# marthinwurer/gcmiipy

Measured on AMD Instinct MI355X. Metric: cell-updates/s (C-grid Matsuno step), higher is better.
Workload: dtype f64; 1 GPU; 2-D shallow water + theta + viscosity + van-Leer tracer, 4096x2048 fp64 (BASELINE configs[2]); variant=fused, decomposition=1 latitude band(s)

## Files before the change

### gcmiipy_amd/_lib.py

```python
import ctypes as C
import os

_HERE = os.path.dirname(os.path.abspath(__file__))
LIB_PATH = os.environ.get("GCMCORE_LIB", os.path.join(_HERE, "lib", "libgcmcore.so"))

ABI_VERSION = 1

SW2D, SW2D_TEMP, PE2D, PE25D = 1, 2, 3, 4
P, U, V, T, Q = 0, 1, 2, 3, 4
TRACER_NONE, TRACER_UPWIND, TRACER_VANLEER = 0, 1, 2
VARIANT_AUTO, VARIANT_STAGED, VARIANT_FUSED = 0, 1, 2
F64, F32 = 0, 1
MAX_TRACERS = 16
TRACER_STATS_WORDS = 6
CLIM_WORDS3, CLIM_WORDS2 = 10, 2
SW2D_PLAN_WORDS = 9
PHASE_HELD_SUAREZ, PHASE_MOIST, PHASE_CLIMATE, PHASE_TRACER_FORCING = range(4)
PHASE_PLAN_WORDS = 5
ADV_UPWIND, ADV_FV_UPWIND, ADV_FV_PLAIN, ADV_VANLEER, ADV_MOMENTUM = range(5)
DIAG_ANY_NAN, DIAG_MAX_U, DIAG_MEAN_P, DIAG_SUM_P, DIAG_MIN_U, DIAG_MAX_V, DIAG_MIN_V = range(7)
DIAG_TV_P, DIAG_TV_U, DIAG_TV_V, DIAG_TV_T, DIAG_TV_Q = range(7, 12)
INT_SPU, INT_PIT, INT_PN, INT_PHI, INT_PGFU = range(5)
FL_VAN_LEER, FL_CALC_R, FL_DONOR_FLUX, FL_DONOR_ADVECTION = range(4)
OP1D_ADVEC_Q, OP1D_CALC_PU, OP1D_UN_PU, OP1D_ADVEC_P, OP1D_ADVEC_PU, OP1D_ADVEC_T, OP1D_PGF = range(7)
# ... 63 lines not shown
class TracerForcing(C.Structure):
    _fields_ = [("source", C.c_double), ("decay", C.c_double), ("pin_value", C.c_double),
                ("emission", _dp), ("pin_mask", C.POINTER(C.c_ubyte))]


_H = C.c_void_p
SYMBOLS = {
    "gcm_abi_version": (C.c_int, []),
    "gcm_device_count": (C.c_int, []),
    "gcm_build_info": (C.c_char_p, []),
    "gcm_exner_table": (C.c_int, [_dp]),
    "gcm_filter_plan": (C.c_int, [C.c_int, C.POINTER(C.c_uint), C.c_int]),
    "gcm_create": (C.c_int, [C.POINTER(Config), C.POINTER(_H)]),
    "gcm_destroy": (C.c_int, [_H]),
    "gcm_last_error": (C.c_char_p, [_H]),
    "gcm_set_state": (C.c_int, [_H] + [C.c_void_p] * 5),
    "gcm_get_state": (C.c_int, [_H] + [C.c_void_p] * 5),
    "gcm_members": (C.c_int, [_H]),
    "gcm_set_member": (C.c_int, [_H, C.c_int] + [C.c_void_p] * 5),
    "gcm_get_member": (C.c_int, [_H, C.c_int] + [C.c_void_p] * 5),
    "gcm_diag_members": (C.c_int, [_H, C.c_int, _dp, C.c_int]),
    "gcm_step": (C.c_int, [_H, C.c_int, C.c_double]),
    "gcm_sw2d_plan": (C.c_int, [_H, C.c_int, C.POINTER(C.c_int), C.c_int]),
    "gcm_pe25d_phase_geometry": (C.c_int, [C.c_int] * 7 + [C.POINTER(C.c_int), C.c_int]),
    "gcm_pe25d_phase_plan": (C.c_int, [_H, C.c_int, C.c_int, C.c_int, C.POINTER(C.c_int), C.c_int]),
    "gcm_half_step": (C.c_int, [_H, C.c_int, C.c_double]),
    "gcm_end_step": (C.c_int, [_H, C.c_double]),
    "gcm_end_step_begin": (C.c_int, [_H, C.c_double]),
    "gcm_end_step_finish": (C.c_int, [_H, C.c_double]),
    "gcm_get_star": (C.c_int, [_H] + [C.c_void_p] * 5),
    "gcm_set_star": (C.c_int, [_H] + [C.c_void_p] * 5),
    "gcm_diag": (C.c_int, [_H, C.c_int, _dp]),
    "gcm_energy": (C.c_int, [_H, _dp, C.c_int, _dp]),
    "gcm_stats": (C.c_int, [_H, _dp, C.c_int, _dp]),
    "gcm_flux_limiter": (C.c_int, [C.c_int, C.c_int, C.c_void_p, C.c_void_p, C.c_double, C.c_double, C.c_void_p]),
    "gcm_polar_filter": (C.c_int, [_H, C.c_int, C.c_void_p, C.c_void_p]),
    "gcm_get_intermediate": (C.c_int, [_H, C.c_int, C.c_void_p]),
    "gcm_set_ground": (C.c_int, [_H, C.c_void_p]),
    "gcm_get_ground": (C.c_int, [_H, C.c_void_p]),
    "gcm_grey_radiation": (C.c_int, [_H] + [C.c_double] * 4 + [_dp, _dp, C.c_void_p, C.c_void_p]),
    "gcm_solar_step": (C.c_int, [_H] + [C.c_double] * 5 + [_dp, _dp]),
    "gcm_set_physics": (C.c_int, [_H, C.c_void_p]),
    "gcm_get_utc": (C.c_int, [_H, _dp]),
    "gcm_set_held_suarez": (C.c_int, [_H, C.POINTER(HeldSuarez)]),
    "gcm_held_suarez_on": (C.c_int, [_H]),
    "gcm_held_suarez_step": (C.c_int, [_H, C.c_double, C.POINTER(HeldSuarez)]),
# ... 117 lines not shown
```

### gcmiipy_amd/core.py

```python
import collections
import ctypes as C

import numpy as np

from . import _lib
from ._lib import lib


class GcmError(RuntimeError):
    pass


def _check(rc, h=None):
    if rc == _lib.OK:
        return
    msg = lib.gcm_last_error(h).decode() if (h or rc) else ""
    if rc == _lib.ERR_ARG:
        raise ValueError(msg or "gcmcore: bad argument")
    raise GcmError("gcmcore error %d: %s" % (rc, msg))


def _count(n, h):
    if n < 0:
        _check(n, h)
# ... 539 lines not shown
                out[i] = k
        return out

    def set_tracer_scheme(self, scheme):
        scheme = tracer_scheme_id(scheme)
        _check(lib.gcm_set_tracer_scheme(self._h, scheme), self._h)
        self.options["tracer_scheme"] = scheme

    @property
    def tracer_scheme(self):
        return _count(lib.gcm_tracer_scheme(self._h), self._h)

    @property
    def band_tracer_rows(self):
        return _count(lib.gcm_band_tracer_rows(self._h), self._h)

    @property
    def tracer_count(self):
        return _count(lib.gcm_tracer_count(self._h), self._h)

    def step(self, nsteps, dt):
        _check(lib.gcm_step(self._h, int(nsteps), float(dt)), self._h)

    def sw2d_plan(self, nsteps):
        out = (C.c_int * _lib.SW2D_PLAN_WORDS)()
        _check(lib.gcm_sw2d_plan(self._h, int(nsteps), out, _lib.SW2D_PLAN_WORDS), self._h)
        return dict(variant={_lib.VARIANT_FUSED: "fused", _lib.VARIANT_STAGED: "staged"}[out[0]],
                    rows_per_band=out[1], cols=out[2], strip=out[3], strip2=out[4], two_step_launches=out[5],
                    single_step_launches=out[6], preload=bool(out[7]), stream=bool(out[8]))

    def phase_plan(self, phase, rows=None, accumulate=True):
        out = (C.c_int * _lib.PHASE_PLAN_WORDS)()
        _check(lib.gcm_pe25d_phase_plan(self._h, phase_id(phase), -1 if rows is None else int(rows), int(bool(accumulate)),
                                        out, _lib.PHASE_PLAN_WORDS), self._h)
        return _phase_dict(phase_id(phase), out)

    def half_step(self, stage, dt):
        _check(lib.gcm_half_step(self._h, int(stage), float(dt)), self._h)

    def end_step(self, dt):
        _check(lib.gcm_end_step(self._h, float(dt)), self._h)

    def end_step_begin(self, dt):
        _check(lib.gcm_end_step_begin(self._h, float(dt)), self._h)

    def end_step_finish(self, dt):
# ... 323 lines not shown
```

### gcmiipy_amd/csrc/gcm_handle.h

```cpp
#pragma once
#include "../../include/gcmcore.h"

#include <hip/hip_runtime.h>

#include <algorithm>
#include <cstdio>
#include <string>
#include <vector>

#include "pe25d_kernels.h"
#include "sw2d_kernels.h"

struct GcmBandExchange {
    gcm_exchange xch{};
    bool set = false, primed = false;
    bool inflight = false;
    bool overlap = false;
    hipEvent_t ev_pack = nullptr, ev_comm = nullptr;
    bool join_pending = false;
    bool on_comm = false;
};

struct GcmTiming {
    bool on = false;
// ... 19 lines not shown
    hipStream_t stream = nullptr;
    std::string err;
    std::vector<void *> allocs;

    double *cur[GCM_NFIELDS] = {}, *nxt[GCM_NFIELDS] = {}, *star[GCM_NFIELDS] = {};
    double *geo = nullptr, *irho = nullptr, *sst = nullptr, *qtmp = nullptr;
    bool has[GCM_NFIELDS] = {};
    double *exner_tab = nullptr;
    int G = gcm::kGhost;
    int since_exchange = 0;
    bool ghosts_current = false;
    bool star_valid = false;
    bool launch_refused = false;
    hipStream_t comm = nullptr;
    double *snap[GCM_NFIELDS] = {};
    int snap_since_exchange = 0;
    int variant = GCM_VARIANT_FUSED;
    int rows_per_band = 32;
    int M = 1;
    long mstride = 0;
    bool f32 = false;
    int esz = 8;
    int cols = 1;
    double *staging = nullptr;
    int staging_members = 0;

    double *diag_dev = nullptr;
    static constexpr int kDiagBlocks = 512;

    GcmTiming time;
    gcm::Pe25d *pe = nullptr;
    GcmBandExchange band;
    GcmPhases phases;
};

#define HIPCHK(h, call)                                                                    \
    do {                                                                                   \
        hipError_t e_ = (call);                                                            \
        if (e_ != hipSuccess) {                                                            \
            char b_[512];                                                                  \
            snprintf(b_, sizeof b_, "%s failed: %s (%s:%d)", #call, hipGetErrorString(e_), \
                     __FILE__, __LINE__);                                                  \
            (h)->err = b_;                                                                 \
            return GCM_ERR_HIP;                                                            \
        }                                                                                  \
    } while (0)
// ... 53 lines not shown
```

### gcmiipy_amd/csrc/gcmcore.hip

```cpp
#include <cmath>
#include <cstdlib>
#include <cstring>

#include "gcm_handle.h"

using namespace gcm;

std::string &gcm_create_error() {
    thread_local std::string e;
    return e;
}

static int alloc_field(gcm_handle *h, double **p) {
    static const long skew_unit = getenv("GCM_ALLOC_SKEW") ? atol(getenv("GCM_ALLOC_SKEW")) : 256;
    const size_t n = all_members_elems(h);
    const size_t skew = (size_t)(skew_unit > 0 ? skew_unit : 0) * (h->allocs.size() % 16) / h->esz;
    void *d = nullptr;
    HIPCHK(h, hipMalloc(&d, (n + skew) * h->esz));
    HIPCHK(h, hipMemsetAsync(d, 0, (n + skew) * h->esz, h->stream));
    h->allocs.push_back(d);
    *p = at(h, (double *)d, (long)(skew + (size_t)h->G * h->W));
    return GCM_OK;
}

// ... 109 lines not shown
            if (cfg->tracer < 0 || cfg->tracer > GCM_TRACER_VANLEER)
                return bail(GCM_ERR_ARG, "gcm_create: bad tracer");
            h->has[GCM_U] = h->has[GCM_V] = h->has[GCM_P] = true;
            h->has[GCM_T] = temp;
            h->has[GCM_Q] = temp && cfg->tracer != GCM_TRACER_NONE;
            h->variant = cfg->variant == GCM_VARIANT_AUTO ? GCM_VARIANT_FUSED : cfg->variant;
            if (h->variant != GCM_VARIANT_FUSED && h->variant != GCM_VARIANT_STAGED)
                return bail(GCM_ERR_ARG, "gcm_create: bad variant");
            for (int f = 0; f < GCM_NFIELDS; ++f) {
                if (!h->has[f]) continue;
                if ((rc = alloc_field(h, &h->cur[f]))) return bail(rc, "");
                if ((rc = alloc_field(h, &h->nxt[f]))) return bail(rc, "");
                if (f != GCM_Q && (rc = alloc_field(h, &h->star[f]))) return bail(rc, "");
            }
            if (temp) {
                if ((rc = alloc_field(h, &h->geo))) return bail(rc, "");
                if ((rc = alloc_field(h, &h->irho))) return bail(rc, "");
                if ((rc = alloc_field(h, &h->sst))) return bail(rc, "");
            }
            if (h->has[GCM_Q] && (rc = alloc_field(h, &h->qtmp))) return bail(rc, "");
            if (temp && !upload_exner_table(h)) return bail(GCM_ERR_HIP, "gcm_create: exner table upload failed");
            const int tr = h->has[GCM_Q] ? cfg->tracer : 0;
            if (h->f32) h->cols = sw2d_fused_cols<float>(h->W, h->H, temp, tr, h->wrap, h->M);
            h->rows_per_band = h->f32 ? sw2d_fused_rows_per_band<float>(h->W, h->H, temp, tr, h->wrap, h->M, h->cols)
                                      : sw2d_fused_rows_per_band<double>(h->W, h->H, temp, tr, h->wrap, h->M);
            break;
        }
        case GCM_PE2D: {
            if (!(cfg->dx > 0)) return bail(GCM_ERR_ARG, "gcm_create: dx must be > 0");
            if (cfg->nranks != 1)
                return bail(GCM_ERR_UNSUPPORTED, "gcm_create: GCM_PE2D has no latitude-band mode");
            h->variant = GCM_VARIANT_STAGED;
            for (int f = 0; f < GCM_NFIELDS; ++f) {
                h->has[f] = true;
                if ((rc = alloc_field(h, &h->cur[f]))) return bail(rc, "");
                if ((rc = alloc_field(h, &h->nxt[f]))) return bail(rc, "");
                if ((rc = alloc_field(h, &h->star[f]))) return bail(rc, "");
            }
            if (!upload_exner_table(h)) return bail(GCM_ERR_HIP, "gcm_create: exner table upload failed");
            break;
        }
        case GCM_PE25D: {
            std::string msg;
            h->pe = pe25d_create(*cfg, h->stream, &msg);
            if (!h->pe) return bail(msg.find("hip") == 0 ? GCM_ERR_HIP : GCM_ERR_ARG, msg);
            h->has[GCM_P] = h->has[GCM_U] = h->has[GCM_V] = h->has[GCM_T] = h->has[GCM_Q] = true;
            break;
        }
// ... 123 lines not shown
    a.inv_dx2 = 1.0 / (h->cfg.dx * h->cfg.dx);
    a.h_dx = 0.5 / h->cfg.dx;
    a.dtdx = dt / h->cfg.dx;
    a.g_dx = 9.8 / h->cfg.dx;
    a.mu_dx2 = (18.5 * 1e-6) * 287.0 / (h->cfg.dx * h->cfg.dx);
    a.inv_dx2_ = a.inv_dx2;
    return a;
}

static void run_derive(const gcm_handle *h, const Sw2dArgs &a, hipStream_t s) {
    if (h->f32) launch_sw2d_derive(narrow_args(a), s);
    else launch_sw2d_derive(a, s);
}
static void run_stage(const gcm_handle *h, const Sw2dArgs &a, bool temp, hipStream_t s) {
    if (h->f32) launch_sw2d_stage(narrow_args(a), temp, s);
    else launch_sw2d_stage(a, temp, s);
}
static void run_tracer_axis(const gcm_handle *h, const Sw2dArgs &a, int axis, bool limit, const double *q_in,
                            double *q_out, hipStream_t s) {
    if (h->f32) launch_tracer_axis(narrow_args(a), axis, limit, (const float *)q_in, (float *)q_out, s);
    else launch_tracer_axis(a, axis, limit, q_in, q_out, s);
}
static bool run_fused(const gcm_handle *h, const Sw2dArgs &a, bool temp, int tracer, hipStream_t s) {
    return h->f32 ? launch_sw2d_fused(narrow_args(a), temp, tracer, s, h->cols) : launch_sw2d_fused(a, temp, tracer, s);
}
static bool run_fused2(const gcm_handle *h, const Sw2dArgs &a, hipStream_t s) {
    return h->f32 ? launch_sw2d_fused2(narrow_args(a), s) : launch_sw2d_fused2(a, s);
}

int launch_status(gcm_handle *h) {
    const hipError_t e = hipGetLastError();
    if (h->launch_refused) {
        h->launch_refused = false;
        return fail(h, GCM_ERR_HIP, std::string("sw2d fused kernel: launch refused") +
                                        (e != hipSuccess ? std::string(": ") + hipGetErrorString(e) : std::string()));
    }
    HIPCHK(h, e);
    return GCM_OK;
}

void swap_state(gcm_handle *h) {
    for (int f = 0; f < GCM_NFIELDS; ++f) std::swap(h->cur[f], h->nxt[f]);
    h->ghosts_current = false;
}

static void tick(gcm_handle *h, hipStream_t s) {
    if (h->time.on && h->time.used < h->time.ev.size()) (void)hipEventRecord(h->time.ev[h->time.used++], s);
// ... 104 lines not shown
                h->launch_refused = true;
                return launch_status(h);
            }
            swap_state(h);
            n0 += 2;
        }
    }
    for (int n = n0; n < nsteps; ++n) {
        const int e = step_extra_rows(h);
        step_rows(h, dt, -e, h->H + e, h->stream);
        swap_state(h);
        if (!h->wrap) ++h->since_exchange;
    }
    h->star_valid = false;
    return launch_status(h);
}

int gcm_sw2d_plan(gcm_handle *h, int nsteps, int *out, int nout) {
    if (!h || h->pe || nsteps < 0 || !out || nout < GCM_SW2D_PLAN_WORDS) return GCM_ERR_ARG;
    const bool fused = h->variant == GCM_VARIANT_FUSED;
    const bool temp = h->cfg.model == GCM_SW2D_TEMP;
    const int pairs = steps_in_pairs(h) ? nsteps / 2 : 0;
    const int e = step_extra_rows(h);
    Sw2dFusedForm f{false, false};
    if (fused)
        f = sw2d_fused_form(temp, h->has[GCM_Q] ? h->cfg.tracer : 0, h->rows_per_band, h->W, h->H + 2 * e, h->M, h->esz);
    out[0] = h->variant;
    out[1] = fused ? h->rows_per_band : 0;
    out[2] = fused ? h->cols : 0;
    out[3] = fused ? sw2d_fused_strip_cols(h->cols) : 0;
    out[4] = fused ? kStrip2Cols : 0;
    out[5] = pairs;
    out[6] = nsteps - 2 * pairs;
    out[7] = f.preload;
    out[8] = f.stream;
    return GCM_OK;
}

int gcm_step_interior(gcm_handle *h, double dt, void *stream) {
    if (!h) return GCM_ERR_ARG;
    if (h->pe) return pe25d_step_part(h->pe, 0, dt, (hipStream_t)stream, &h->err);
    if (h->wrap) return fail(h, GCM_ERR_STATE, "step_interior: handle is not a latitude band");
    if (h->G != kGhost) return fail(h, GCM_ERR_STATE, "step_interior: halo_steps > 1 steps through gcm_step");
    step_rows(h, dt, kGhost, h->H - kGhost, (hipStream_t)stream);
    return launch_status(h);
}

int gcm_step_boundary(gcm_handle *h, double dt, void *stream) {
    if (!h) return GCM_ERR_ARG;
    if (h->pe) return pe25d_step_part(h->pe, 1, dt, (hipStream_t)stream, &h->err);
    if (h->wrap) return fail(h, GCM_ERR_STATE, "step_boundary: handle is not a latitude band");
    hipStream_t s = (hipStream_t)stream;
    if (h->H <= 2 * kGhost) {
        step_rows(h, dt, 0, h->H, s);
    } else {
        step_rows(h, dt, 0, kGhost, s);
        step_rows(h, dt, h->H - kGhost, h->H, s);
    }
    swap_state(h);
// ... 204 lines not shown
```

### gcmiipy_amd/csrc/sw2d_impl.h

```cpp
#pragma once
#include <hip/hip_runtime.h>

#include <cstdlib>
#include <type_traits>

#include "gcm_math.h"
#include "sw2d_kernels.h"

namespace gcm {

__device__ __forceinline__ long row_off(int j, int H, int W, bool wrap) {
    if (wrap) {
        j %= H;
        if (j < 0) j += H;
    }
    return (long)j * W;
}

template <typename T>
__device__ __forceinline__ Sw2dArgsT<T> member_args(const Sw2dArgsT<T> &a0, int m) {
    Sw2dArgsT<T> a = a0;
    const long o = (long)m * a0.mstride;
    auto mv = [o](auto *p) { return p ? p + o : p; };
    a.bu = mv(a.bu); a.bv = mv(a.bv); a.bp = mv(a.bp); a.bt = mv(a.bt); a.bq = mv(a.bq);
// ... 171 lines not shown
    t.du = adv_vel_u(R0.u, uw, ue, RM.u, RP.u, R0.v, vw, RP.v, vsw, h_dx) +
           geo_grad(ge, R0.g, g_dx);
    t.dv = adv_vel_v(R0.v, vw, ve, RM.v, RP.v, R0.u, RM.u, uw, usw, h_dx) +
           geo_grad(RP.g, R0.g, g_dx);
    if (TEMP) {
        const T vis = visc_u(R0.u, uw, ue, RM.u, RP.u, mu_dx2) * R0.irho;
        t.du -= vis;
        t.dv -= vis;
    }
    t.dp = adv_geo(R0.u, uw, R0.v, RM.v, R0.p, pw, pe, RM.p, RP.p, h_dx);
    t.dst = T(0.0);
    if (TEMP) {
        const T stw = from_west(R0.st), ste = from_east(R0.st);
        t.dst = adv_geo(R0.u, uw, R0.v, RM.v, R0.st, stw, ste, RM.st, RP.st, h_dx);
    }
    return t;
}

template <typename T>
struct Raw {
    T u, v, p, t, q;
};

template <typename T, bool TEMP, int TRACER, bool WRAPJ, bool STREAM = false, int CPL = 1>
struct FusedCtx {
    using Real = std::conditional_t<CPL == 2, f32x2, T>;
    using V = Real;
    const Sw2dArgsT<T> &a;
    const double *tab;
    int ci, col, ja, jb;
    bool store_lane;
    V f0_prev;

    __device__ __forceinline__ Raw<V> load(int j) const {
        const long o = row_off(j, a.H, a.W, WRAPJ) + ci;
        Raw<V> r;
        if constexpr (CPL == 2) {
            auto ld = [o](const T *p) {
                const f32x2 *q = (const f32x2 *)(p + o);
                return STREAM ? __builtin_nontemporal_load(q) : *q;
            };
            r.u = ld(a.bu);
            r.v = ld(a.bv);
            r.p = ld(a.bp);
            r.t = TEMP ? ld(a.bt) : V(0.0f);
            r.q = TRACER ? ld(a.bq) : V(0.0f);
        } else if (STREAM) {
            r.u = __builtin_nontemporal_load(&a.bu[o]);
            r.v = __builtin_nontemporal_load(&a.bv[o]);
            r.p = __builtin_nontemporal_load(&a.bp[o]);
            r.t = TEMP ? __builtin_nontemporal_load(&a.bt[o]) : T(0.0);
            r.q = TRACER ? __builtin_nontemporal_load(&a.bq[o]) : T(0.0);
        } else {
            r.u = a.bu[o];
            r.v = a.bv[o];
            r.p = a.bp[o];
            r.t = TEMP ? a.bt[o] : T(0.0);
            r.q = TRACER ? a.bq[o] : T(0.0);
        }
        return r;
    }

    template <bool FETCH = true>
    __device__ __forceinline__ void iter(int r, Row<V> &BM, Row<V> &B0, Row<V> &BP, Row<V> &SN, Row<V> &SM,
                                         Row<V> &S0, Raw<V> &nxt, V &qmm, V &qm, V &q0, V &qp) {
        const V dt = V(a.dt), g_dx = V(a.g_dx), h_dx = V(a.h_dx), mu_dx2 = V(a.mu_dx2), dtdx = V(a.dtdx);
        {
            const Tend<V> t = tendencies<TEMP>(BM, B0, BP, g_dx, h_dx, mu_dx2);
            const V us = B0.u - dt * t.du;
            const V vs = B0.v - dt * t.dv;
            const V ps = B0.p - dt * t.dp;
            V ts = V(0.0), rps = V(0.0);
            if (TEMP) {
                rps = rcp(ps);
                ts = (B0.st - dt * t.dst) * rps;
            }
            make_row_r<TEMP>(SN, us, vs, ps, ts, tab, rps);
        }
        V f0_cur = V(0.0);
        if (TRACER && r >= ja) f0_cur = face_flux<TRACER == 2>(BM.v, qmm, qm, q0, qp, dtdx);
        if (r >= ja + 1) {
            const Tend<V> t = tendencies<TEMP>(SM, S0, SN, g_dx, h_dx, mu_dx2);
            const V un = BM.u - dt * t.du;
            const V vn = BM.v - dt * t.dv;
            const V pn = BM.p - dt * t.dp;
            V tn = V(0.0), qn = V(0.0);
            if (TEMP) tn = (BM.st - dt * t.dst) * rcp(pn);
            if (TRACER) {
                const V qs = qm - f0_cur + f0_prev;
                const V qs_w = from_west(qs), qs_e = from_east(qs);
                const V qs_ee = from_east(qs_e);
                const V f1 = face_flux<TRACER == 2>(BM.u, qs_w, qs, qs_e, qs_ee, dtdx);
                qn = qs - f1 + from_west(f1);
            }
            if (store_lane) {
                const long o = (long)(r - 1) * a.W + col;
                if constexpr (CPL == 2) {
                    auto st = [o](T *p, V x) { *(V *)(p + o) = x; };
                    st(a.ou, un);
                    st(a.ov, vn);
                    st(a.op, pn);
                    if (TEMP) st(a.ot, tn);
                    if (TRACER) st(a.oq, qn);
                } else {
                    a.ou[o] = un;
                    a.ov[o] = vn;
                    a.op[o] = pn;
                    if (TEMP) a.ot[o] = tn;
                    if (TRACER) a.oq[o] = qn;
                }
            }
        }
        f0_prev = f0_cur;
        make_row<TEMP>(BM, nxt.u, nxt.v, nxt.p, nxt.t, tab);
        if (TRACER) {
            qmm = qm;
            qm = q0;
            q0 = qp;
            qp = nxt.q;
        }
        if (FETCH && r + 3 <= jb + 1) nxt = load(r + 3);
    }
};

template <int N, int PRE, class Ctx, typename T = typename Ctx::Real>
__device__ __forceinline__ void preloaded_iters(Ctx &c, const Raw<T> (&pre)[PRE + 4], Row<T> &A, Row<T> &B, Row<T> &C,
                                                Row<T> &X, Row<T> &Y, Row<T> &Z, Raw<T> &nxt, T &qmm, T &qm, T &q0,
                                                T &qp) {
    if constexpr (N < PRE + 2) {
        const int r = c.ja - 1 + N;
        if (r > c.jb) return;
        c.template iter<false>(r, A, B, C, X, Y, Z, nxt, qmm, qm, q0, qp);
        if constexpr (N < PRE) nxt = pre[N + 4];
        preloaded_iters<N + 1, PRE>(c, pre, B, C, A, Y, Z, X, nxt, qmm, qm, q0, qp);
    }
}

template <typename T, bool TEMP, int TRACER, bool WRAPJ, int PRE = 0, bool STREAM = false, int CPL = 1>
__global__ __launch_bounds__(64, (CPL == 2 && TRACER != 0) ? 3 : 1) void sw2d_fused_kernel(Sw2dArgsT<T> a0) {
    using Ctx = FusedCtx<T, TEMP, TRACER, WRAPJ, STREAM, CPL>;
    using V = typename Ctx::Real;
    constexpr int kCols = sw2d_fused_strip_cols(CPL);
    const int W = a0.W;
    const int lane = threadIdx.x;
    const int strips = (W + kCols - 1) / kCols;
    const int per_xcd = gridDim.x / 8;
    int tile = (blockIdx.x % 8) * per_xcd + blockIdx.x / 8;
    int member = 0;
    if (a0.members > 1) {
        const int per_member = strips * ((a0.j1 - a0.j0 + a0.rows_per_band - 1) / a0.rows_per_band);
        member = tile / per_member;
        if (member >= a0.members) return;
        tile -= member * per_member;
    }
    const int band = tile / strips;
    const int i0 = (tile - band * strips) * kCols;
    const Sw2dArgsT<T> a = member_args(a0, member);
    __shared__ double tab[kExnerTabDoubles];
    if (TEMP) {
        for (int k = 0; k < kExnerTabDoubles / 64; ++k) tab[lane + 64 * k] = a.exner_tab[lane + 64 * k];
        __syncthreads();
    }
    Ctx c{a, tab};
    c.ja = a.j0 + band * a.rows_per_band;
    c.jb = min(c.ja + a.rows_per_band, a.j1);
    if (c.ja >= c.jb) return;
    c.col = i0 - 2 * CPL + CPL * lane;
    c.ci = c.col % W;
    if (c.ci < 0) c.ci += W;
    c.store_lane = lane >= 2 && lane < 62 && c.col < W;
    c.f0_prev = V(0.0);
    const int ja = c.ja, jb = c.jb;

    Row<V> A, B, C, X, Y, Z;
    if constexpr (PRE > 0) {
        Raw<V> pre[PRE + 4];
#pragma unroll
        for (int n = 0; n < PRE + 4; ++n) pre[n] = c.load(min(ja - 2 + n, jb + 1));
        make_row<TEMP>(A, pre[0].u, pre[0].v, pre[0].p, pre[0].t, tab);
        make_row<TEMP>(B, pre[1].u, pre[1].v, pre[1].p, pre[1].t, tab);
        make_row<TEMP>(C, pre[2].u, pre[2].v, pre[2].p, pre[2].t, tab);
        V qmm = V(0.0), qm = pre[0].q, q0 = pre[1].q, qp = pre[2].q;
        Raw<V> nxt = pre[3];
        X = Y = Z = A;
        preloaded_iters<0, PRE>(c, pre, A, B, C, X, Y, Z, nxt, qmm, qm, q0, qp);
        return;
    }
    Raw<V> x = c.load(ja - 2);
    make_row<TEMP>(A, x.u, x.v, x.p, x.t, tab);
    V qmm = V(0.0), qm = x.q;
    x = c.load(ja - 1);
    make_row<TEMP>(B, x.u, x.v, x.p, x.t, tab);
    V q0 = x.q;
    x = c.load(ja);
    make_row<TEMP>(C, x.u, x.v, x.p, x.t, tab);
    V qp = x.q;
    Raw<V> nxt = c.load(ja + 1);
    X = Y = Z = A;

    for (int r = ja - 1; r <= jb; r += 3) {
        c.iter(r, A, B, C, X, Y, Z, nxt, qmm, qm, q0, qp);
        if (r + 1 > jb) break;
        c.iter(r + 1, B, C, A, Y, Z, X, nxt, qmm, qm, q0, qp);
        if (r + 2 > jb) break;
        c.iter(r + 2, C, A, B, Z, X, Y, nxt, qmm, qm, q0, qp);
    }
}

// ... 100 lines not shown
    make_row<false>(A1, pre[0].u, pre[0].v, pre[0].p, T(0.0), nullptr);
    make_row<false>(B1, pre[1].u, pre[1].v, pre[1].p, T(0.0), nullptr);
    make_row<false>(C1, pre[2].u, pre[2].v, pre[2].p, T(0.0), nullptr);
    X1 = Y1 = Z1 = A2 = B2 = C2 = X2 = Y2 = Z2 = A1;
    fused2_iters<0, RPB>(c, pre, A1, B1, C1, X1, Y1, Z1, A2, B2, C2, X2, Y2, Z2);
}

template <typename T>
bool launch_sw2d_fused2(const Sw2dArgsT<T> &a, hipStream_t s) {
    if (!sw2d_fused2_serves(a.wrap_j, a.j0, a.j1, a.H, a.rows_per_band)) return false;
    const int strips = (a.W + kStrip2Cols - 1) / kStrip2Cols;
    const int bands = (a.H + a.rows_per_band - 1) / a.rows_per_band;
    dim3 g((unsigned)(((long)strips * bands * a.members + 7) / 8 * 8));
    Sw2dArgsT<T> arg = a;
    void *params[] = {&arg};
    const bool ens = a.members > 1;
    const void *fn = a.rows_per_band == 2 ? (ens ? (const void *)sw2d_fused2_kernel<T, 2, true> : (const void *)sw2d_fused2_kernel<T, 2, false>)
                   : a.rows_per_band == 3 ? (ens ? (const void *)sw2d_fused2_kernel<T, 3, true> : (const void *)sw2d_fused2_kernel<T, 3, false>)
                                          : (ens ? (const void *)sw2d_fused2_kernel<T, 4, true> : (const void *)sw2d_fused2_kernel<T, 4, false>);
    return hipLaunchKernel(fn, g, dim3(64), params, 0, s) == hipSuccess;
}

template <typename T, bool TEMP, int TRACER, int CPL = 1>
static const void *fused_fn(bool wrap, bool stream) {
    if (stream)
        return wrap ? (const void *)sw2d_fused_kernel<T, TEMP, TRACER, true, 0, true, CPL>
                    : (const void *)sw2d_fused_kernel<T, TEMP, TRACER, false, 0, true, CPL>;
    return wrap ? (const void *)sw2d_fused_kernel<T, TEMP, TRACER, true, 0, false, CPL>
                : (const void *)sw2d_fused_kernel<T, TEMP, TRACER, false, 0, false, CPL>;
}

template <typename T, int CPL>
static const void *fused_kernel_ptr_c(bool temp, int tracer, bool wrap, bool preload, bool stream) {
    if (!temp) {
        if (preload)
            return wrap ? (const void *)sw2d_fused_kernel<T, false, 0, true, kPreloadRows, false, CPL>
                        : (const void *)sw2d_fused_kernel<T, false, 0, false, kPreloadRows, false, CPL>;
        return fused_fn<T, false, 0, CPL>(wrap, stream);
    }
    if (tracer == 0) return fused_fn<T, true, 0, CPL>(wrap, stream);
    if (tracer == 1) return fused_fn<T, true, 1, CPL>(wrap, stream);
    return fused_fn<T, true, 2, CPL>(wrap, stream);
}

template <typename T>
static const void *fused_kernel_ptr(bool temp, int tracer, bool wrap, bool preload = false, bool stream = false,
                                    int cols = 1) {
    if constexpr (std::is_same_v<T, float>)
        if (cols == 2) return fused_kernel_ptr_c<T, 2>(temp, tracer, wrap, preload, stream);
    return fused_kernel_ptr_c<T, 1>(temp, tracer, wrap, preload, stream);
}

template <typename T>
int sw2d_fused_rows_per_band(int W, int H, bool temp, int tracer, bool wrap, int members, int cols) {
    if (const char *e = getenv("GCM_FUSED_ROWS")) {
        int v = atoi(e);
        if (v > 0) return v;
    }
    int waves_per_cu = 12, cus = 256, dev = 0;
    hipDeviceProp_t prop;
    if (hipGetDevice(&dev) == hipSuccess && hipGetDeviceProperties(&prop, dev) == hipSuccess)
        cus = prop.multiProcessorCount;
    int nb = 0;
    if (hipOccupancyMaxActiveBlocksPerMultiprocessor(&nb, fused_kernel_ptr<T>(temp, tracer, wrap, false, false, cols), 64,
                                                     0) == hipSuccess && nb > 0)
        waves_per_cu = nb;
    const long slots = (long)waves_per_cu * cus;
    const long M = members < 1 ? 1 : members;
    const long strips = (W + sw2d_fused_strip_cols(cols) - 1) / sw2d_fused_strip_cols(cols);
    auto waves = [&](int rpb) { return M * strips * ((H + rpb - 1) / rpb); };
    if (waves(8) < slots) {
        long rpb = M * H * strips / (5L * cus);
        if (!temp && M > 1 && rpb > kPreloadRows) rpb = kPreloadRows;
        return (int)(rpb < 2 ? 2 : rpb > 8 ? 8 : rpb);
    }
    long rounds = (waves(64) + slots - 1) / slots;
    long bands = rounds * slots / (strips * M);
    if (bands < 1) bands = 1;
    long rpb = (H + bands - 1) / bands;
    return (int)(rpb < 8 ? 8 : rpb);
}

template <typename T>
int sw2d_fused_cols(int W, int H, bool temp, int tracer, bool wrap, int members) {
    if (!std::is_same_v<T, float> || W % 2) return 1;
    if (const char *e = getenv("GCM_SW2D_F32_COLS")) return e[0] == '1' ? 1 : 2;
    int waves_per_cu = 12, cus = 256, dev = 0, nb = 0;
    hipDeviceProp_t prop;
    if (hipGetDevice(&dev) == hipSuccess && hipGetDeviceProperties(&prop, dev) == hipSuccess)
        cus = prop.multiProcessorCount;
    if (hipOccupancyMaxActiveBlocksPerMultiprocessor(&nb, fused_kernel_ptr<T>(temp, tracer, wrap), 64, 0) == hipSuccess &&
        nb > 0)
        waves_per_cu = nb;
    const long strips = (W + kStripCols - 1) / kStripCols;
    const long waves8 = (long)(members < 1 ? 1 : members) * strips * ((H + 7) / 8);
    return waves8 < (long)waves_per_cu * cus ? 1 : 2;
}

template <typename T>
bool launch_sw2d_fused(const Sw2dArgsT<T> &a, bool temp, int tracer, hipStream_t s, int cols) {
    if (a.j1 <= a.j0) return true;
    const int strips = (a.W + sw2d_fused_strip_cols(cols) - 1) / sw2d_fused_strip_cols(cols);
    const int bands = (a.j1 - a.j0 + a.rows_per_band - 1) / a.rows_per_band;
    dim3 g((unsigned)(((long)strips * bands * a.members + 7) / 8 * 8));
    Sw2dArgsT<T> arg = a;
    void *params[] = {&arg};
    const Sw2dFusedForm f = sw2d_fused_form(temp, tracer, a.rows_per_band, a.W, a.j1 - a.j0, a.members, (long)sizeof(T));
    return hipLaunchKernel(fused_kernel_ptr<T>(temp, tracer, a.wrap_j != 0, f.preload, f.stream, cols), g, dim3(64), params, 0, s) == hipSuccess;
}

template <typename T>
__global__ void copy_rows_kernel(T *dst, const T *src, long n) {
    long i = (long)blockIdx.x * blockDim.x + threadIdx.x;
    const long stride = (long)gridDim.x * blockDim.x;
    for (; i < n; i += stride) dst[i] = src[i];
}

template <typename T>
void launch_copy_rows(T *dst, const T *src, int W, int nrows, hipStream_t s) {
    const long n = (long)W * nrows;
    if (n <= 0) return;
    int blocks = (int)((n + 255) / 256);
    if (blocks > 1024) blocks = 1024;
    hipLaunchKernelGGL(copy_rows_kernel<T>, dim3(blocks), dim3(256), 0, s, dst, src, n);
}

#define GCM_SW2D_INSTANTIATE(T)                                                                                   \
    template void launch_sw2d_stage<T>(const Sw2dArgsT<T> &, bool, hipStream_t);                                 \
    template void launch_sw2d_derive<T>(const Sw2dArgsT<T> &, hipStream_t);                                      \
    template void launch_tracer_axis<T>(const Sw2dArgsT<T> &, int, bool, const T *, T *, hipStream_t);           \
    template bool launch_sw2d_fused<T>(const Sw2dArgsT<T> &, bool, int, hipStream_t, int);                       \
    template int sw2d_fused_rows_per_band<T>(int, int, bool, int, bool, int, int);                              \
    template int sw2d_fused_cols<T>(int, int, bool, int, bool, int);                                            \
    template bool launch_sw2d_fused2<T>(const Sw2dArgsT<T> &, hipStream_t);                                      \
    template void launch_copy_rows<T>(T *, const T *, int, int, hipStream_t);

}
```

### gcmiipy_amd/csrc/sw2d_kernels.h

```cpp
#pragma once
#include <hip/hip_runtime.h>

namespace gcm {

constexpr int kExnerTabDoubles = 256;
constexpr int kGhost = 2;
constexpr int kStripCols = 60;

constexpr int kStrip2Cols = 56;
constexpr int kPreloadRows = 4;

constexpr int sw2d_fused_strip_cols(int cols) { return cols * kStripCols; }
inline bool sw2d_fused2_serves(int wrap_j, int j0, int j1, int H, int rows_per_band) {
    return wrap_j && j0 == 0 && j1 == H && rows_per_band >= 2 && rows_per_band <= 4;
}
struct Sw2dFusedForm {
    bool preload, stream;
};
inline Sw2dFusedForm sw2d_fused_form(bool temp, int tracer, int rows_per_band, long W, long rows, long members,
                                     long esz) {
    const int nfields = 3 + (temp ? 1 : 0) + (tracer ? 1 : 0);
    const bool preload = !temp && rows_per_band <= kPreloadRows;
    return {preload, !preload && W * rows * members * esz * nfields > (256L << 20)};
}

template <typename T>
struct Sw2dArgsT {
    const T *bu, *bv, *bp, *bt, *bq;
    const T *su, *sv, *sp, *st;
    const T *sgeo, *sirho, *sst;
    T *ou, *ov, *op, *ot, *oq;
    T *dgeo, *dirho, *dst;
    const double *exner_tab;
    int W, H;
    int wrap_j;
    int j0, j1;
    int rows_per_band;
    int members;
    long mstride;
    T dt, dx, inv_dx, dx2, inv_dx2;
    T h_dx;
    T dtdx;
    T g_dx, mu_dx2, inv_dx2_;
};
using Sw2dArgs = Sw2dArgsT<double>;

inline Sw2dArgsT<float> narrow_args(const Sw2dArgs &a) {
    Sw2dArgsT<float> f{};
    auto cp = [](auto *p) { return (float *)p; };
    f.bu = cp(a.bu); f.bv = cp(a.bv); f.bp = cp(a.bp); f.bt = cp(a.bt); f.bq = cp(a.bq);
    f.su = cp(a.su); f.sv = cp(a.sv); f.sp = cp(a.sp); f.st = cp(a.st);
    f.sgeo = cp(a.sgeo); f.sirho = cp(a.sirho); f.sst = cp(a.sst);
    f.ou = cp(a.ou); f.ov = cp(a.ov); f.op = cp(a.op); f.ot = cp(a.ot); f.oq = cp(a.oq);
    f.dgeo = cp(a.dgeo); f.dirho = cp(a.dirho); f.dst = cp(a.dst);
    f.exner_tab = a.exner_tab;
    f.W = a.W; f.H = a.H; f.wrap_j = a.wrap_j; f.j0 = a.j0; f.j1 = a.j1;
    f.rows_per_band = a.rows_per_band; f.members = a.members; f.mstride = a.mstride;
    f.dt = (float)a.dt; f.dx = (float)a.dx; f.inv_dx = (float)a.inv_dx; f.dx2 = (float)a.dx2;
    f.inv_dx2 = (float)a.inv_dx2; f.h_dx = (float)a.h_dx; f.dtdx = (float)a.dtdx; f.g_dx = (float)a.g_dx;
    f.mu_dx2 = (float)a.mu_dx2; f.inv_dx2_ = (float)a.inv_dx2_;
    return f;
}

template <typename T> void launch_sw2d_stage(const Sw2dArgsT<T> &a, bool temp, hipStream_t s);
template <typename T> void launch_sw2d_derive(const Sw2dArgsT<T> &a, hipStream_t s);
template <typename T>
void launch_tracer_axis(const Sw2dArgsT<T> &a, int axis, bool limit, const T *q_in, T *q_out, hipStream_t s);
template <typename T>
bool launch_sw2d_fused(const Sw2dArgsT<T> &a, bool temp, int tracer, hipStream_t s, int cols = 1);
template <typename T>
int sw2d_fused_rows_per_band(int W, int H, bool temp, int tracer, bool wrap, int members = 1, int cols = 1);
template <typename T> int sw2d_fused_cols(int W, int H, bool temp, int tracer, bool wrap, int members);
template <typename T> bool launch_sw2d_fused2(const Sw2dArgsT<T> &a, hipStream_t s);
void launch_narrow(float *dst, long pitch, const double *src, long n, int M, hipStream_t s);
void launch_widen(double *dst, const float *src, long pitch, long n, int M, hipStream_t s);

void launch_pe2d_stage(const double *const base[5], const double *const stage[5], double *const out[5],
                       const double *exner_tab, int W, int H, double dt, double dx, hipStream_t s);

void build_exner_table(double *tab);

template <typename T> void launch_copy_rows(T *dst, const T *src, int W, int nrows, hipStream_t s);

struct SegCopy {
    double *dst[44];
    const double *src[44];
    long n[44];
    int nseg;
};
void launch_seg_copy(const SegCopy &c, hipStream_t s, hipEvent_t stop = nullptr);

}
```

### include/gcmcore.h

```cpp
#ifndef GCMCORE_H
#define GCMCORE_H

#include <stddef.h>
#include <stdint.h>

#ifdef __cplusplus
extern "C" {
#endif

#define GCM_ABI_VERSION 1

typedef struct gcm_handle gcm_handle;

typedef enum {
    GCM_OK = 0,
    GCM_ERR_ARG = -1,
    GCM_ERR_HIP = -2,
    GCM_ERR_NODEVICE = -3,
    GCM_ERR_STATE = -4,
    GCM_ERR_UNSUPPORTED = -5
} gcm_status;

typedef enum {
    GCM_SW2D = 1,
// ... 54 lines not shown
int gcm_device_count(void);
const char *gcm_build_info(void);
int gcm_exner_table(double *out256);
int gcm_filter_plan(int n, unsigned *out, int cap);

int gcm_create(const gcm_config *cfg, gcm_handle **out);
int gcm_destroy(gcm_handle *h);
const char *gcm_last_error(const gcm_handle *h);

int gcm_set_state(gcm_handle *h, const double *p, const double *u, const double *v,
                  const double *t, const double *q);
int gcm_get_state(gcm_handle *h, double *p, double *u, double *v, double *t, double *q);

int gcm_members(const gcm_handle *h);
int gcm_set_member(gcm_handle *h, int m, const double *p, const double *u, const double *v,
                   const double *t, const double *q);
int gcm_get_member(gcm_handle *h, int m, double *p, double *u, double *v, double *t, double *q);

int gcm_step(gcm_handle *h, int nsteps, double dt);

#define GCM_SW2D_PLAN_WORDS 9
int gcm_sw2d_plan(gcm_handle *h, int nsteps, int *out, int nout);

typedef enum { GCM_PHASE_HELD_SUAREZ = 0, GCM_PHASE_MOIST = 1, GCM_PHASE_CLIMATE = 2, GCM_PHASE_TRACER_FORCING = 3 } gcm_pe25d_phase;
#define GCM_PHASE_PLAN_WORDS 5
int gcm_pe25d_phase_geometry(int phase, int W, int rows, int L, int cus, int elem_bytes, int accumulate, int *out, int nout);
int gcm_pe25d_phase_plan(gcm_handle *h, int phase, int rows, int accumulate, int *out, int nout);

int gcm_half_step(gcm_handle *h, int stage, double dt);
int gcm_get_star(gcm_handle *h, double *p, double *u, double *v, double *t, double *q);
int gcm_set_star(gcm_handle *h, const double *p, const double *u, const double *v,
                 const double *t, const double *q);

#define GCM_MAX_TRACERS 16
int gcm_set_tracers(gcm_handle *h, int n, const double *c);
int gcm_get_tracers(gcm_handle *h, int which, double *c);
int gcm_tracer_count(const gcm_handle *h);
int gcm_set_tracer_scheme(gcm_handle *h, int scheme);
int gcm_tracer_scheme(const gcm_handle *h);
int gcm_set_band_tracers(gcm_handle *h, int n);
int gcm_set_band_tracer_rows(gcm_handle *h, int rows);
int gcm_band_tracer_rows(const gcm_handle *h);
#define GCM_TRACER_STATS_WORDS 6
int gcm_tracer_stats(gcm_handle *h, int which, int with_q, double *out, int cap);
typedef struct gcm_tracer_forcing {
    double source, decay, pin_value;
// ... 204 lines not shown
```

Measured before the change: 58.65 billion cell-updates/s.

## Add deep-prefetch fused march for large fp64 temp+tracer shallow-water steps

Adds a DEPTH=3 variant of the fused row-marching kernel that keeps three rows of loads in flight (prefetching five rows ahead), unrolls the march by three, and writes rows through buffer stores with an out-of-range offset instead of a branch on the store lane. It is chosen automatically for single-member fp64 temp configurations large enough to use the streaming form, and can also be forced with an environment variable. Band sizing is reworked for this path to fill whole rounds of occupancy slots, with bands capped at 96 rows and launch bounds set for two waves per unit. The intent is to hide global-memory latency in the bandwidth-bound march. In exchange it uses more registers and lowers occupancy, and it adds a kernel instantiation and a query API.

```diff
diff --git a/gcmiipy_amd/_lib.py b/gcmiipy_amd/_lib.py
--- a/gcmiipy_amd/_lib.py
+++ b/gcmiipy_amd/_lib.py
@@ -109,6 +109,7 @@
     "gcm_diag_members": (C.c_int, [_H, C.c_int, _dp, C.c_int]),
     "gcm_step": (C.c_int, [_H, C.c_int, C.c_double]),
     "gcm_sw2d_plan": (C.c_int, [_H, C.c_int, C.POINTER(C.c_int), C.c_int]),
+    "gcm_sw2d_fused_depth": (C.c_int, [_H]),
     "gcm_pe25d_phase_geometry": (C.c_int, [C.c_int] * 7 + [C.POINTER(C.c_int), C.c_int]),
     "gcm_pe25d_phase_plan": (C.c_int, [_H, C.c_int, C.c_int, C.c_int, C.POINTER(C.c_int), C.c_int]),
     "gcm_half_step": (C.c_int, [_H, C.c_int, C.c_double]),
diff --git a/gcmiipy_amd/core.py b/gcmiipy_amd/core.py
--- a/gcmiipy_amd/core.py
+++ b/gcmiipy_amd/core.py
@@ -585,6 +585,11 @@
     def step(self, nsteps, dt):
         _check(lib.gcm_step(self._h, int(nsteps), float(dt)), self._h)
 
+    def sw2d_fused_depth(self):
+        d = lib.gcm_sw2d_fused_depth(self._h)
+        _check(min(d, 0), self._h)
+        return d
+
     def sw2d_plan(self, nsteps):
         out = (C.c_int * _lib.SW2D_PLAN_WORDS)()
         _check(lib.gcm_sw2d_plan(self._h, int(nsteps), out, _lib.SW2D_PLAN_WORDS), self._h)
diff --git a/gcmiipy_amd/csrc/gcm_handle.h b/gcmiipy_amd/csrc/gcm_handle.h
--- a/gcmiipy_amd/csrc/gcm_handle.h
+++ b/gcmiipy_amd/csrc/gcm_handle.h
@@ -65,6 +65,7 @@
     bool f32 = false;
     int esz = 8;
     int cols = 1;
+    int depth_pin = 0;
     double *staging = nullptr;
     int staging_members = 0;
 
diff --git a/gcmiipy_amd/csrc/gcmcore.hip b/gcmiipy_amd/csrc/gcmcore.hip
--- a/gcmiipy_amd/csrc/gcmcore.hip
+++ b/gcmiipy_amd/csrc/gcmcore.hip
@@ -155,8 +155,10 @@
             if (temp && !upload_exner_table(h)) return bail(GCM_ERR_HIP, "gcm_create: exner table upload failed");
             const int tr = h->has[GCM_Q] ? cfg->tracer : 0;
             if (h->f32) h->cols = sw2d_fused_cols<float>(h->W, h->H, temp, tr, h->wrap, h->M);
+            if (const char *e = getenv("GCM_SW2D_DEPTH"))
+                if (temp && !h->f32 && (e[0] == '1' || e[0] == '3') && !e[1]) h->depth_pin = e[0] - '0';
             h->rows_per_band = h->f32 ? sw2d_fused_rows_per_band<float>(h->W, h->H, temp, tr, h->wrap, h->M, h->cols)
-                                      : sw2d_fused_rows_per_band<double>(h->W, h->H, temp, tr, h->wrap, h->M);
+                                      : sw2d_fused_rows_per_band<double>(h->W, h->H, temp, tr, h->wrap, h->M, 1, h->depth_pin);
             break;
         }
         case GCM_PE2D: {
@@ -326,7 +328,7 @@
     else launch_tracer_axis(a, axis, limit, q_in, q_out, s);
 }
 static bool run_fused(const gcm_handle *h, const Sw2dArgs &a, bool temp, int tracer, hipStream_t s) {
-    return h->f32 ? launch_sw2d_fused(narrow_args(a), temp, tracer, s, h->cols) : launch_sw2d_fused(a, temp, tracer, s);
+    return h->f32 ? launch_sw2d_fused(narrow_args(a), temp, tracer, s, h->cols) : launch_sw2d_fused(a, temp, tracer, s, 1, h->depth_pin);
 }
 static bool run_fused2(const gcm_handle *h, const Sw2dArgs &a, hipStream_t s) {
     return h->f32 ? launch_sw2d_fused2(narrow_args(a), s) : launch_sw2d_fused2(a, s);
@@ -477,9 +479,9 @@
     const bool temp = h->cfg.model == GCM_SW2D_TEMP;
     const int pairs = steps_in_pairs(h) ? nsteps / 2 : 0;
     const int e = step_extra_rows(h);
-    Sw2dFusedForm f{false, false};
+    Sw2dFusedForm f{false, false, 1};
     if (fused)
-        f = sw2d_fused_form(temp, h->has[GCM_Q] ? h->cfg.tracer : 0, h->rows_per_band, h->W, h->H + 2 * e, h->M, h->esz);
+        f = sw2d_fused_form(temp, h->has[GCM_Q] ? h->cfg.tracer : 0, h->rows_per_band, h->W, h->H + 2 * e, h->M, h->esz, h->depth_pin);
     out[0] = h->variant;
     out[1] = fused ? h->rows_per_band : 0;
     out[2] = fused ? h->cols : 0;
@@ -490,6 +492,14 @@
     out[7] = f.preload;
     out[8] = f.stream;
     return GCM_OK;
+}
+
+int gcm_sw2d_fused_depth(gcm_handle *h) {
+    if (!h || h->pe) return GCM_ERR_ARG;
+    if (h->variant != GCM_VARIANT_FUSED) return 0;
+    const int e = step_extra_rows(h);
+    return sw2d_fused_form(h->cfg.model == GCM_SW2D_TEMP, h->has[GCM_Q] ? h->cfg.tracer : 0, h->rows_per_band, h->W,
+                           h->H + 2 * e, h->M, h->esz, h->depth_pin).depth;
 }
 
 int gcm_step_interior(gcm_handle *h, double dt, void *stream) {
diff --git a/gcmiipy_amd/csrc/sw2d_impl.h b/gcmiipy_amd/csrc/sw2d_impl.h
--- a/gcmiipy_amd/csrc/sw2d_impl.h
+++ b/gcmiipy_amd/csrc/sw2d_impl.h
@@ -217,6 +217,19 @@
     T u, v, p, t, q;
 };
 
+constexpr unsigned kNoStore = 0x80000000u;
+__device__ __forceinline__ void store_row_lanes(double *row, int W, unsigned lane_off, double x) {
+    typedef unsigned int u32x2 __attribute__((ext_vector_type(2)));
+    const __amdgpu_buffer_rsrc_t rs = __builtin_amdgcn_make_buffer_rsrc(row, 0, W * 8, 0x00020000);
+    __builtin_amdgcn_raw_buffer_store_b64(__builtin_bit_cast(u32x2, x), rs, (int)lane_off, 0, 0);
+}
+
+__device__ __forceinline__ double own_copy(double x) {
+    double y;
+    asm volatile("v_mov_b64 %0, %1" : "=v"(y) : "v"(x) : "memory");
+    return y;
+}
+
 template <typename T, bool TEMP, int TRACER, bool WRAPJ, bool STREAM = false, int CPL = 1>
 struct FusedCtx {
     using Real = std::conditional_t<CPL == 2, f32x2, T>;
@@ -256,7 +269,7 @@
         return r;
     }
 
-    template <bool FETCH = true>
+    template <bool FETCH = true, int AHEAD = 3, int LEAD = -1, bool ROWBUF = false>
     __device__ __forceinline__ void iter(int r, Row<V> &BM, Row<V> &B0, Row<V> &BP, Row<V> &SN, Row<V> &SM,
                                          Row<V> &S0, Raw<V> &nxt, V &qmm, V &qm, V &q0, V &qp) {
         const V dt = V(a.dt), g_dx = V(a.g_dx), h_dx = V(a.h_dx), mu_dx2 = V(a.mu_dx2), dtdx = V(a.dtdx);
@@ -273,8 +286,8 @@
             make_row_r<TEMP>(SN, us, vs, ps, ts, tab, rps);
         }
         V f0_cur = V(0.0);
-        if (TRACER && r >= ja) f0_cur = face_flux<TRACER == 2>(BM.v, qmm, qm, q0, qp, dtdx);
-        if (r >= ja + 1) {
+        if (TRACER && (LEAD < 0 ? r >= ja : LEAD >= 1)) f0_cur = face_flux<TRACER == 2>(BM.v, qmm, qm, q0, qp, dtdx);
+        if (LEAD < 0 ? r >= ja + 1 : LEAD >= 2) {
             const Tend<V> t = tendencies<TEMP>(SM, S0, SN, g_dx, h_dx, mu_dx2);
             const V un = BM.u - dt * t.du;
             const V vn = BM.v - dt * t.dv;
@@ -288,7 +301,15 @@
                 const V f1 = face_flux<TRACER == 2>(BM.u, qs_w, qs, qs_e, qs_ee, dtdx);
                 qn = qs - f1 + from_west(f1);
             }
-            if (store_lane) {
+            if constexpr (ROWBUF) {
+                const long o = (long)(r - 1) * a.W;
+                const unsigned lane_off = store_lane ? (unsigned)col * 8u : kNoStore;
+                store_row_lanes(a.ou + o, a.W, lane_off, un);
+                store_row_lanes(a.ov + o, a.W, lane_off, vn);
+                store_row_lanes(a.op + o, a.W, lane_off, pn);
+                if (TEMP) store_row_lanes(a.ot + o, a.W, lane_off, tn);
+                if (TRACER) store_row_lanes(a.oq + o, a.W, lane_off, qn);
+            } else if (store_lane) {
                 const long o = (long)(r - 1) * a.W + col;
                 if constexpr (CPL == 2) {
                     auto st = [o](T *p, V x) { *(V *)(p + o) = x; };
@@ -307,14 +328,23 @@
             }
         }
         f0_prev = f0_cur;
-        make_row<TEMP>(BM, nxt.u, nxt.v, nxt.p, nxt.t, tab);
+        if constexpr (AHEAD == 3) {
+            make_row<TEMP>(BM, nxt.u, nxt.v, nxt.p, nxt.t, tab);
+        } else {
+            make_row<TEMP>(BM, own_copy(nxt.u), own_copy(nxt.v), own_copy(nxt.p), TEMP ? own_copy(nxt.t) : nxt.t, tab);
+        }
         if (TRACER) {
             qmm = qm;
             qm = q0;
             q0 = qp;
-            qp = nxt.q;
-        }
-        if (FETCH && r + 3 <= jb + 1) nxt = load(r + 3);
+            if constexpr (AHEAD == 3) qp = nxt.q;
+            else qp = own_copy(nxt.q);
+        }
+        if constexpr (AHEAD == 3) {
+            if (FETCH && r + 3 <= jb + 1) nxt = load(r + 3);
+        } else {
+            nxt = load(min(r + AHEAD, jb + 1));
+        }
     }
 };
 
@@ -331,8 +361,8 @@
     }
 }
 
-template <typename T, bool TEMP, int TRACER, bool WRAPJ, int PRE = 0, bool STREAM = false, int CPL = 1>
-__global__ __launch_bounds__(64, (CPL == 2 && TRACER != 0) ? 3 : 1) void sw2d_fused_kernel(Sw2dArgsT<T> a0) {
+template <typename T, bool TEMP, int TRACER, bool WRAPJ, int PRE = 0, bool STREAM = false, int CPL = 1, int DEPTH = 1>
+__global__ __launch_bounds__(64, DEPTH == 3 ? 2 : (CPL == 2 && TRACER != 0) ? 3 : 1) void sw2d_fused_kernel(Sw2dArgsT<T> a0) {
     using Ctx = FusedCtx<T, TEMP, TRACER, WRAPJ, STREAM, CPL>;
     using V = typename Ctx::Real;
     constexpr int kCols = sw2d_fused_strip_cols(CPL);
@@ -379,6 +409,29 @@
         Raw<V> nxt = pre[3];
         X = Y = Z = A;
         preloaded_iters<0, PRE>(c, pre, A, B, C, X, Y, Z, nxt, qmm, qm, q0, qp);
+        return;
+    }
+    if constexpr (DEPTH == 3) {
+        static_assert(PRE == 0 && CPL == 1, "the deep march is the rolling form with one column per lane");
+        const Raw<V> w0 = c.load(ja - 2), w1 = c.load(ja - 1), w2 = c.load(ja);
+        Raw<V> n0 = c.load(ja + 1), n1 = c.load(ja + 2), n2 = c.load(min(ja + 3, jb + 1));
+        make_row<TEMP>(A, w0.u, w0.v, w0.p, w0.t, tab);
+        make_row<TEMP>(B, w1.u, w1.v, w1.p, w1.t, tab);
+        make_row<TEMP>(C, w2.u, w2.v, w2.p, w2.t, tab);
+        V qmm = V(0.0), qm = w0.q, q0 = w1.q, qp = w2.q;
+        X = Y = Z = A;
+        c.template iter<true, 5, 0, true>(ja - 1, A, B, C, X, Y, Z, n0, qmm, qm, q0, qp);
+        c.template iter<true, 5, 1, true>(ja, B, C, A, Y, Z, X, n1, qmm, qm, q0, qp);
+        int r = ja + 1;
+        for (; r + 2 <= jb; r += 3) {
+            c.template iter<true, 5, 2, true>(r, C, A, B, Z, X, Y, n2, qmm, qm, q0, qp);
+            c.template iter<true, 5, 2, true>(r + 1, A, B, C, X, Y, Z, n0, qmm, qm, q0, qp);
+            c.template iter<true, 5, 2, true>(r + 2, B, C, A, Y, Z, X, n1, qmm, qm, q0, qp);
+        }
+        if (r <= jb) {
+            c.template iter<false, 3, 2, true>(r, C, A, B, Z, X, Y, n2, qmm, qm, q0, qp);
+            if (r + 1 <= jb) c.template iter<false, 3, 2, true>(r + 1, A, B, C, X, Y, Z, n0, qmm, qm, q0, qp);
+        }
         return;
     }
     Raw<V> x = c.load(ja - 2);
@@ -525,7 +578,16 @@
 }
 
 template <typename T, bool TEMP, int TRACER, int CPL = 1>
-static const void *fused_fn(bool wrap, bool stream) {
+static const void *fused_fn(bool wrap, bool stream, int depth = 1) {
+    if constexpr (std::is_same_v<T, double> && TEMP && CPL == 1) {
+        if (depth == 3) {
+            if (stream)
+                return wrap ? (const void *)sw2d_fused_kernel<T, TEMP, TRACER, true, 0, true, CPL, 3>
+                            : (const void *)sw2d_fused_kernel<T, TEMP, TRACER, false, 0, true, CPL, 3>;
+            return wrap ? (const void *)sw2d_fused_kernel<T, TEMP, TRACER, true, 0, false, CPL, 3>
+                        : (const void *)sw2d_fused_kernel<T, TEMP, TRACER, false, 0, false, CPL, 3>;
+        }
+    }
     if (stream)
         return wrap ? (const void *)sw2d_fused_kernel<T, TEMP, TRACER, true, 0, true, CPL>
                     : (const void *)sw2d_fused_kernel<T, TEMP, TRACER, false, 0, true, CPL>;
@@ -534,44 +596,55 @@
 }
 
 template <typename T, int CPL>
-static const void *fused_kernel_ptr_c(bool temp, int tracer, bool wrap, bool preload, bool stream) {
+static const void *fused_kernel_ptr_c(bool temp, int tracer, bool wrap, bool preload, bool stream, int depth) {
     if (!temp) {
         if (preload)
             return wrap ? (const void *)sw2d_fused_kernel<T, false, 0, true, kPreloadRows, false, CPL>
                         : (const void *)sw2d_fused_kernel<T, false, 0, false, kPreloadRows, false, CPL>;
         return fused_fn<T, false, 0, CPL>(wrap, stream);
     }
-    if (tracer == 0) return fused_fn<T, true, 0, CPL>(wrap, stream);
-    if (tracer == 1) return fused_fn<T, true, 1, CPL>(wrap, stream);
-    return fused_fn<T, true, 2, CPL>(wrap, stream);
+    if (tracer == 0) return fused_fn<T, true, 0, CPL>(wrap, stream, depth);
+    if (tracer == 1) return fused_fn<T, true, 1, CPL>(wrap, stream, depth);
+    return fused_fn<T, true, 2, CPL>(wrap, stream, depth);
 }
 
 template <typename T>
 static const void *fused_kernel_ptr(bool temp, int tracer, bool wrap, bool preload = false, bool stream = false,
-                                    int cols = 1) {
+                                    int cols = 1, int depth = 1) {
     if constexpr (std::is_same_v<T, float>)
-        if (cols == 2) return fused_kernel_ptr_c<T, 2>(temp, tracer, wrap, preload, stream);
-    return fused_kernel_ptr_c<T, 1>(temp, tracer, wrap, preload, stream);
-}
-
-template <typename T>
-int sw2d_fused_rows_per_band(int W, int H, bool temp, int tracer, bool wrap, int members, int cols) {
+        if (cols == 2) return fused_kernel_ptr_c<T, 2>(temp, tracer, wrap, preload, stream, 1);
+    return fused_kernel_ptr_c<T, 1>(temp, tracer, wrap, preload, stream, depth);
+}
+
+constexpr int kDeepMaxRows = 96;
+template <typename T>
+int sw2d_fused_rows_per_band(int W, int H, bool temp, int tracer, bool wrap, int members, int cols, int depth_pin) {
     if (const char *e = getenv("GCM_FUSED_ROWS")) {
         int v = atoi(e);
         if (v > 0) return v;
     }
-    int waves_per_cu = 12, cus = 256, dev = 0;
+    const long M = members < 1 ? 1 : members;
+    const Sw2dFusedForm form = sw2d_fused_form(temp, tracer, kPreloadRows + 1, W, H, M, (long)sizeof(T), depth_pin);
+    const bool deep = form.depth == 3;
+    int waves_per_cu = deep ? 8 : 12, cus = 256, dev = 0;
     hipDeviceProp_t prop;
     if (hipGetDevice(&dev) == hipSuccess && hipGetDeviceProperties(&prop, dev) == hipSuccess)
         cus = prop.multiProcessorCount;
     int nb = 0;
-    if (hipOccupancyMaxActiveBlocksPerMultiprocessor(&nb, fused_kernel_ptr<T>(temp, tracer, wrap, false, false, cols), 64,
-                                                     0) == hipSuccess && nb > 0)
+    if (hipOccupancyMaxActiveBlocksPerMultiprocessor(&nb, fused_kernel_ptr<T>(temp, tracer, wrap, false, deep && form.stream, cols, form.depth),
+                                                     64, 0) == hipSuccess && nb > 0)
         waves_per_cu = nb;
     const long slots = (long)waves_per_cu * cus;
-    const long M = members < 1 ? 1 : members;
     const long strips = (W + sw2d_fused_strip_cols(cols) - 1) / sw2d_fused_strip_cols(cols);
     auto waves = [&](int rpb) { return M * strips * ((H + rpb - 1) / rpb); };
+    if (deep && waves(8) >= slots) {
+        for (long rounds = 1;; ++rounds) {
+            long bands = rounds * slots / (strips * M);
+            if (bands < 1) bands = 1;
+            const long rpb = (H + bands - 1) / bands;
+            if (rpb <= kDeepMaxRows || bands >= H) return (int)(rpb < 8 ? 8 : rpb);
+        }
+    }
     if (waves(8) < slots) {
         long rpb = M * H * strips / (5L * cus);
         if (!temp && M > 1 && rpb > kPreloadRows) rpb = kPreloadRows;
@@ -601,15 +674,15 @@
 }
 
 template <typename T>
-bool launch_sw2d_fused(const Sw2dArgsT<T> &a, bool temp, int tracer, hipStream_t s, int cols) {
+bool launch_sw2d_fused(const Sw2dArgsT<T> &a, bool temp, int tracer, hipStream_t s, int cols, int depth_pin) {
     if (a.j1 <= a.j0) return true;
     const int strips = (a.W + sw2d_fused_strip_cols(cols) - 1) / sw2d_fused_strip_cols(cols);
     const int bands = (a.j1 - a.j0 + a.rows_per_band - 1) / a.rows_per_band;
     dim3 g((unsigned)(((long)strips * bands * a.members + 7) / 8 * 8));
     Sw2dArgsT<T> arg = a;
     void *params[] = {&arg};
-    const Sw2dFusedForm f = sw2d_fused_form(temp, tracer, a.rows_per_band, a.W, a.j1 - a.j0, a.members, (long)sizeof(T));
-    return hipLaunchKernel(fused_kernel_ptr<T>(temp, tracer, a.wrap_j != 0, f.preload, f.stream, cols), g, dim3(64), params, 0, s) == hipSuccess;
+    const Sw2dFusedForm f = sw2d_fused_form(temp, tracer, a.rows_per_band, a.W, a.j1 - a.j0, a.members, (long)sizeof(T), depth_pin);
+    return hipLaunchKernel(fused_kernel_ptr<T>(temp, tracer, a.wrap_j != 0, f.preload, f.stream, cols, f.depth), g, dim3(64), params, 0, s) == hipSuccess;
 }
 
 template <typename T>
@@ -632,8 +705,8 @@
     template void launch_sw2d_stage<T>(const Sw2dArgsT<T> &, bool, hipStream_t);                                 \
     template void launch_sw2d_derive<T>(const Sw2dArgsT<T> &, hipStream_t);                                      \
     template void launch_tracer_axis<T>(const Sw2dArgsT<T> &, int, bool, const T *, T *, hipStream_t);           \
-    template bool launch_sw2d_fused<T>(const Sw2dArgsT<T> &, bool, int, hipStream_t, int);                       \
-    template int sw2d_fused_rows_per_band<T>(int, int, bool, int, bool, int, int);                              \
+    template bool launch_sw2d_fused<T>(const Sw2dArgsT<T> &, bool, int, hipStream_t, int, int);                  \
+    template int sw2d_fused_rows_per_band<T>(int, int, bool, int, bool, int, int, int);                         \
     template int sw2d_fused_cols<T>(int, int, bool, int, bool, int);                                            \
     template bool launch_sw2d_fused2<T>(const Sw2dArgsT<T> &, hipStream_t);                                      \
     template void launch_copy_rows<T>(T *, const T *, int, int, hipStream_t);
diff --git a/gcmiipy_amd/csrc/sw2d_kernels.h b/gcmiipy_amd/csrc/sw2d_kernels.h
--- a/gcmiipy_amd/csrc/sw2d_kernels.h
+++ b/gcmiipy_amd/csrc/sw2d_kernels.h
@@ -16,12 +16,15 @@
 }
 struct Sw2dFusedForm {
     bool preload, stream;
+    int depth;
 };
 inline Sw2dFusedForm sw2d_fused_form(bool temp, int tracer, int rows_per_band, long W, long rows, long members,
-                                     long esz) {
+                                     long esz, int pin = 0) {
     const int nfields = 3 + (temp ? 1 : 0) + (tracer ? 1 : 0);
     const bool preload = !temp && rows_per_band <= kPreloadRows;
-    return {preload, !preload && W * rows * members * esz * nfields > (256L << 20)};
+    const bool stream = !preload && W * rows * members * esz * nfields > (256L << 20);
+    const bool deep = temp && esz == 8 && !preload && W < (1L << 27) && (pin ? pin == 3 : stream && members == 1);
+    return {preload, stream, deep ? 3 : 1};
 }
 
 template <typename T>
@@ -67,9 +70,11 @@
 template <typename T>
 void launch_tracer_axis(const Sw2dArgsT<T> &a, int axis, bool limit, const T *q_in, T *q_out, hipStream_t s);
 template <typename T>
-bool launch_sw2d_fused(const Sw2dArgsT<T> &a, bool temp, int tracer, hipStream_t s, int cols = 1);
+bool launch_sw2d_fused(const Sw2dArgsT<T> &a, bool temp, int tracer, hipStream_t s, int cols = 1,
+                       int depth_pin = 0);
 template <typename T>
-int sw2d_fused_rows_per_band(int W, int H, bool temp, int tracer, bool wrap, int members = 1, int cols = 1);
+int sw2d_fused_rows_per_band(int W, int H, bool temp, int tracer, bool wrap, int members = 1, int cols = 1,
+                             int depth_pin = 0);
 template <typename T> int sw2d_fused_cols(int W, int H, bool temp, int tracer, bool wrap, int members);
 template <typename T> bool launch_sw2d_fused2(const Sw2dArgsT<T> &a, hipStream_t s);
 void launch_narrow(float *dst, long pitch, const double *src, long n, int M, hipStream_t s);
diff --git a/include/gcmcore.h b/include/gcmcore.h
--- a/include/gcmcore.h
+++ b/include/gcmcore.h
@@ -100,6 +100,8 @@
 #define GCM_SW2D_PLAN_WORDS 9
 int gcm_sw2d_plan(gcm_handle *h, int nsteps, int *out, int nout);
 
+int gcm_sw2d_fused_depth(gcm_handle *h);
+
 typedef enum { GCM_PHASE_HELD_SUAREZ = 0, GCM_PHASE_MOIST = 1, GCM_PHASE_CLIMATE = 2, GCM_PHASE_TRACER_FORCING = 3 } gcm_pe25d_phase;
 #define GCM_PHASE_PLAN_WORDS 5
 int gcm_pe25d_phase_geometry(int phase, int W, int rows, int L, int cus, int elem_bytes, int accumulate, int *out, int nout);
```

Result: faster. 63.95 billion cell-updates/s (median of 6 runs) (+9.0%).
